# mahilab/mahi-mpc

Hardware: AMD Instinct MI355X
Metric: MPC solves/sec (whole node), nx=4 N=30 batch, at 1/2/4/8 MI355X (higher is better)
Workload: dtype f64; 1 GPU; cfg#2: 2-link arm nx=4 nu=2, N=30, h=2 ms, cold-start SQP (exact or Gauss-Newton Hessian: config.hessian) to ||grad||<=1e-8, ||g||<=1e-10; batch_per_gpu=4096, global_batch=4096, horizon=30, kkt_solver=riccati (16 lanes per instance), hessian=exact (Lagrangian, IPOPT's default), init_states=reference cold start V = 0 (MMPC_INIT_ZERO: V not read)

## Files before the change

### mahi-mpc_amd/csrc/sqp_group.h

```cpp
#undef MMPC_GROUP_PASS
#if defined(MMPC_GROUP_BODY_ONLY)
#define MMPC_GROUP_PASS 2
#elif !defined(MMPC_SQP_GROUP_H)
#define MMPC_SQP_GROUP_H
#define MMPC_GROUP_PASS 1
#else
#define MMPC_GROUP_PASS 0
#endif
#if MMPC_GROUP_PASS == 1
#include <type_traits>

#include "models.h"
#include "sqp_lane.h"
#include "sqp_wave.h"

namespace mmpc {

template <class Model>
__host__ __device__ constexpr bool w_struct_zero(int, int) { return false; }
template <>
__host__ __device__ constexpr bool w_struct_zero<TwoLinkArm>(int r, int j) { return (r == 0 && j >= 2) || (r >= 2 && (j == 0 || j >= 4)); }
template <class Model>
struct WPack {
    static constexpr int PK = 0, OVER = 0;
// ... 123 lines not shown
        for (int s = 0; s < (NQ > NA ? NQ : NA); ++s) {
            if (s < NA) t = fma(lFqd[i * NA + s], x[NQ + s] - lxs[NQ + s], t);
            if (s < NQ) t = fma(lFq[i * NQ + s], x[s] - lxs[s], t);
        }
#pragma unroll
        for (int c = 0; c < NU; ++c) t = fma(lFu[i * NU + c], u[c] - lus[c], t);
        xd[NQ + i] = t;
    }
    if (jac) {
#pragma unroll
        for (int i = 0; i < NA * NQ; ++i) Fq[i] = lFq[i];
#pragma unroll
        for (int i = 0; i < NA * NA; ++i) Fqd[i] = lFqd[i];
#pragma unroll
        for (int i = 0; i < NA * NU; ++i) Fu[i] = lFu[i];
    }
}

template <class Model, bool BOUNDED = false, bool XB = false, bool EXACT = false>
__global__ __launch_bounds__(64) void sqp_group_kernel(SolveParams p, GroupWork gw) {
    constexpr bool MEHR = false;
    constexpr bool IB = false;
#endif
#if MMPC_GROUP_PASS != 0
    static_assert(!(BOUNDED && XB), "the interior-point variant handles the control bounds itself");
    static_assert(!MEHR || XB, "the barrier rule belongs to the interior-point variant");
    constexpr int NX = Model::NX, NU = Model::NU, NQ = Model::NQ, NA = NX - NQ, NS = NX + NU, ND = NX + NU;
    constexpr int SQ = NA * NQ > 0 ? NA * NQ : 1;
    constexpr int FQ = NA * NQ, FD = NA * NA, FU = NA * NU;
    static_assert(NQ >= 0 && NA >= NQ, "x = [q; z] with qdot = z[0:NQ]");
    constexpr int G = kGroupLanes;
    extern __shared__ double shm[];
    const int gl = threadIdx.x & (G - 1);
    const int gi = threadIdx.x / G;
    [[maybe_unused]] const int lane0 = threadIdx.x;
    MMPC_PHASE_DECL
    const int gbase = gi * G;
    const int64_t slot = (int64_t)blockIdx.x * p.gpw + gi;
    const bool resume = p.tail_idx != nullptr;
    const bool valid = gi < p.gpw && slot < (resume ? (int64_t)min(*p.tail_count, p.tail_slots) : p.B);
    if (!valid) return;
    const int64_t inst = resume ? (int64_t)p.tail_idx[slot] : slot;
    const int64_t ii = inst;
    const int N = p.N;
    const int NV = NX * (N + 1) + NU * N;
    const double h = p.h;

    constexpr int KC = NX + NU < kGroupLanes ? GroupLaneOps<Model>::doubles : 0;
    double* const sX = shm + gi * group_lds_doubles(NX, NU, NQ, N, BOUNDED, p.is_linear != 0, XB, KC);
    double* const sU = sX + (N + 1) * NX;
    double* const sD = sU + N * NU;
    double* const sDX = sD + (N + 1) * NX;
    double* const sDU = sDX + (N + 1) * NX;
    double* const sF = sDU + N * NU;
    double* const sC = sF + N * NX;
    double* const sFq = sC + N * NX;
    double* const sFqd = sFq + N * FQ;
    double* const sFu = sFqd + N * FD;
    double* const sR = sFu + N * FU;
    double* const sHold = sR + N * NX;
    double* const sLin = sHold + (BOUNDED ? N * NU : 0);
    constexpr int NY = NX + NU;
    constexpr int PK = WPack<Model>::PK;
    constexpr bool WLDS = EXACT && !BOUNDED && !XB && IsControlAffine<Model>::value && PK >= NX && PK <= 2 * NX + NU;
    double* const wK = gw.ws + slot * (int64_t)group_ws_doubles(NX, NU, N, BOUNDED, XB, WLDS, MEHR);
    constexpr int KZ = NX + NU, HW = group_hess_doubles(NX, NU);
    double* const wH = wK + N * NU * (NS + 1);
    double* const sW = sD + NX;
    static_assert(!WLDS || WPack<Model>::OVER <= NX, "the over-read of the last W record stays inside sDU");
    if constexpr (WLDS) {
        if (gl < WPack<Model>::OVER) sW[N * PK + gl] = 0.0;
    }
    constexpr int NR = NS + NU + 1;
    double* const wRel = wH + N * HW;
    bool w_zeros_stored = false;
    double* const sZl = wRel;
    double* const sZu = sZl + N * NY;
    double* const sSg = sZu + N * NY;
    double* const sBb = sSg + N * NY;
    double* const sZg = sBb + N * NY;
    [[maybe_unused]] double* const sCl = sZg + N * NY;
    [[maybe_unused]] double* const sCu = sCl + N * NY;
    constexpr int VL = 2 + NU, VC = NU * (NU + 1) / 2, VS = VC + NU, VR = VL * G + VS;
    [[maybe_unused]] double* const sVr = sCu + N * NY;
    const double* const trg = p.traj + ii * (int64_t)N * NX;

    const double* w = p.weights + ii * p.w_stride;
    double Q[NX], R[NU], Rm[NU], up[NU];
#pragma unroll
    for (int r = 0; r < NX; ++r) Q[r] = w[r];
#pragma unroll
    for (int c = 0; c < NU; ++c) {
        R[c] = w[NX + c];
        Rm[c] = w[NX + NU + c];
        up[c] = p.u_prev[ii * NU + c];
    }
    double lbv[NU], ubv[NU];
    load_bounds<NU, BOUNDED, IB>(p, inst, lbv, ubv);
    constexpr bool DIST = (NS < G);
    static_assert(!MEHR || DIST, "Mehrotra's rule: lane-distributed path");
    constexpr bool CAFF = IsControlAffine<Model>::value;
    static_assert(!EXACT || (DIST && HasHess<Model>::value), "exact Hessian: lane-distributed path, model eval_hess");
    const int r = gl;
    const bool lx = r < NX, lu = r >= NX && r < NS, la = r >= NQ && r < NX;
    const int rx = lx ? r : 0;
    const int ru = lu ? r - NX : 0;
    const int ta = la ? r - NQ : 0;
    const double Qr = lx ? w[rx] : 0.0;
    [[maybe_unused]] const double lqd = r < NQ ? 1.0 : 0.0, lad = la ? 1.0 : 0.0;
    const double lxf = lx ? 1.0 : 0.0;
    int wrow = 0;
#pragma unroll
    for (int r2 = 0; r2 < NX; ++r2)
        if (lx && r == r2) wrow = WPack<Model>::col(r2);
    double wm[KZ];
#pragma unroll
    for (int j = 0; j < KZ; ++j) {
        bool nz = false;
#pragma unroll
        for (int r2 = 0; r2 < NX; ++r2)
            if (lx && r == r2 && WPack<Model>::idx(r2, j) >= 0) nz = true;
        wm[j] = wpack_col_rep<Model>(j) < j ? wm[wpack_col_rep<Model>(j)] : (nz ? 1.0 : 0.0);
    }
    const int rq = r < NQ ? r : 0;
    const double Rr = lu ? w[NX + ru] : 0.0;
    double dgx[NS];
#pragma unroll
    for (int j = 0; j < NS; ++j) dgx[j] = (lx && j == r) ? 1.0 : 0.0;
    double lbr = -INFINITY, ubr = INFINITY;
#pragma unroll
    for (int c = 0; c < NU; ++c)
        if (lu && ru == c) {
            lbr = lbv[c];
            ubr = ubv[c];
        }
    double hq[NQ > 0 ? NQ : 1], hrow[NX], qoh[NX], rdg[NU];
#pragma unroll
    for (int z = 0; z < NQ; ++z) hq[z] = (r == NQ + z) ? h : 0.0;
#pragma unroll
    for (int j = 0; j < NX; ++j) {
        hrow[j] = (r < NQ && j == NQ + r) ? h : 0.0;
        qoh[j] = (j == r) ? Qr : 0.0;
    }
#pragma unroll
    for (int c = 0; c < NU; ++c) rdg[c] = (r == NX + c) ? R[c] : 0.0;
    constexpr bool LOPS = KC > 0;
    double* const sKc = sX + group_lds_doubles(NX, NU, NQ, N, BOUNDED, p.is_linear != 0, XB, KC) - KC;
    using LdsB = const __attribute__((address_space(3))) char*;
    using LdsD = const __attribute__((address_space(3))) double*;
    const LdsB shb = (LdsB)shm;
    auto lds = [](LdsB b) { return *(LdsD)b; };
    auto pin = [](LdsB& b) { asm volatile("" : "+v"(b)); };
    [[maybe_unused]] const LdsB iKc = shb + 8 * (int)(sKc - shm), iKz = iKc + 8 * NX;
    [[maybe_unused]] const LdsB iAq = la ? shb + 8 * ((int)(sFq - shm) + ta * NQ) : (r < NQ ? iKc + 8 * ((NX - 1) - (NQ + r)) : iKz);
    [[maybe_unused]] const int zAq = la ? 8 * FQ : 0, zAd = la ? 8 * FD : 0, zBr = la ? 8 * FU : 0;
    [[maybe_unused]] const LdsB iAd = la ? shb + 8 * ((int)(sFqd - shm) + ta * NA) : (r < NQ ? iAq + 8 * NQ : iKz);
    [[maybe_unused]] const LdsB iBr = la ? shb + 8 * ((int)(sFu - shm) + ta * NU) : iKz;
    constexpr bool ACOLP = LOPS && NQ == NA && (NA - 1) * NA < KC;
    [[maybe_unused]] const int zAc = (la || r < NQ) ? 8 * FD : 0;
    [[maybe_unused]] const LdsB iAc = la ? shb + 8 * ((int)(sFqd - shm) + ta) : (r < NQ ? shb + 8 * ((int)(sFq - shm) + rq) : iKc),
                                iAcN = iAc + (N - 1) * zAc;
    if constexpr (LOPS) {
        for (int i = gl; i < KC; i += G) sKc[i] = (i == NX - 1) ? h : 0.0;
    }
    {
        const double* Vin = p.V + ii * (int64_t)NV;
        for (int k = gl; k <= N; k += G) {
#pragma unroll
            for (int r = 0; r < NX; ++r)
                sX[k * NX + r] = (k == 0 || p.init_hold) ? p.x0[ii * NX + r] : (p.init_zero ? 0.0 : Vin[k * ND + r]);
            if (k < N) {
#pragma unroll
                for (int c = 0; c < NU; ++c) {
                    const double v = p.init_zero ? 0.0 : Vin[k * ND + NX + c];
                    sU[k * NU + c] = BOUNDED ? proj(v, lbv[c], ubv[c]) : v;
                }
#pragma unroll
                for (int r = 0; r < NX; ++r) sR[k * NX + r] = trg[k * NX + r];
            }
        }
    }
    const double* const tr = sR;
    double yl[XB ? NY : 1], yu[XB ? NY : 1];
    double mub = (XB && resume) ? p.tail_mub[slot] : kIpMu0;
    if constexpr (XB) {
        load_ip_bounds<NX, NU, IB>(p, inst, yl, yu);
        __builtin_amdgcn_wave_barrier();
        if (resume) {
            const double* const lz = p.tail_lws + (inst >> 6) * p.tail_lws_block + (inst & 63);
            for (int k = gl; k < N; k += G) {
#pragma unroll
                for (int j = 0; j < NY; ++j) {
                    sZl[k * NY + j] = lz[((int64_t)k * p.tail_lws_ss + p.tail_lws_zl + j) * 64];
                    sZu[k * NY + j] = lz[((int64_t)k * p.tail_lws_ss + p.tail_lws_zl + NY + j) * 64];
                }
            }
        } else {
            for (int k = gl; k < N; k += G) {
#pragma unroll
                for (int j = 0; j < NY; ++j) {
                    double& y = j < NX ? sX[(k + 1) * NX + j] : sU[k * NU + j - NX];
                    y = ip_push(y, yl[j], yu[j]);
                    sZl[k * NY + j] = yl[j] > -INFINITY ? 1.0 : 0.0;
                    sZu[k * NY + j] = yu[j] < INFINITY ? 1.0 : 0.0;
                }
            }
        }
    }
    const bool lin = p.is_linear != 0;
    double* const lFq = sLin;
    double* const lFqd = lFq + FQ;
    double* const lFu = lFqd + FD;
    double* const lxd = lFu + FU;
    const double* const lxs = sX;
    if (lin && gl == 0) {
        double acc[NA], x[NX], Fq[SQ], Fqd[FD], Fu[FU];
#pragma unroll
        for (int r = 0; r < NX; ++r) x[r] = p.x0[ii * NX + r];
        Model::eval_acc_jac(x, up, acc, Fq, Fqd, Fu);
#pragma unroll
        for (int i = 0; i < FQ; ++i) lFq[i] = Fq[i];
#pragma unroll
        for (int i = 0; i < FD; ++i) lFqd[i] = Fqd[i];
#pragma unroll
        for (int i = 0; i < FU; ++i) lFu[i] = Fu[i];
#pragma unroll
        for (int i = 0; i < NQ; ++i) lxd[i] = x[NQ + i];
#pragma unroll
        for (int i = 0; i < NA; ++i) lxd[NQ + i] = acc[i];
    }
    __builtin_amdgcn_wave_barrier();
    int status = ST_MAX_ITER;
    int it = 0;
    double kkt = 0.0, mu = resume ? p.tail_mu[slot] : 0.0, pg_prev = (BOUNDED && resume) ? p.tail_mub[slot] : INFINITY;
    bool done = !valid;
    constexpr bool FUSE_FWD = true;
    bool fwd_ready = false;
    double J0n = 0.0, c1n = 0.0, cmaxn = 0.0;
    int nfn = 0;
    MMPC_PHASE(0);
    for (it = resume ? p.tail_it[slot] : 0; !done; ++it) {
        MMPC_PHASE(8);
        __builtin_amdgcn_wave_barrier();
        double J0 = J0n, c1 = c1n, cmax = cmaxn;
        int nonfinite = nfn;
        const bool evalA = !(FUSE_FWD && fwd_ready);
        if (evalA) {
            J0 = 0.0;
            c1 = 0.0;
            cmax = 0.0;
            nonfinite = 0;
            for (int k = gl; k < N; k += G) {
                double x[NX], u[NU], xd[NX], Fq[SQ], Fqd[FD], Fu[FU];
#pragma unroll
                for (int r = 0; r < NX; ++r) x[r] = sX[k * NX + r];
#pragma unroll
                for (int c = 0; c < NU; ++c) u[c] = sU[k * NU + c];
                group_model<Model>(lin, lFq, lFqd, lFu, lxd, lxs, up, x, u, xd, Fq, Fqd, Fu, true);
#pragma unroll
                for (int i = 0; i < FQ; ++i) sFq[k * FQ + i] = h * Fq[i];
#pragma unroll
                for (int i = 0; i < FD; ++i) sFqd[k * FD + i] = h * Fqd[i];
#pragma unroll
                for (int i = 0; i < FU; ++i) sFu[k * FU + i] = h * Fu[i];
#pragma unroll
                for (int r = 0; r < NX; ++r) {
                    const double F = fma(h, xd[r], x[r]);
                    sF[k * NX + r] = F;
                    const double c = F - sX[(k + 1) * NX + r];
                    sC[k * NX + r] = c;
                    cmax = fmax(cmax, fabs(c));
                    c1 += fabs(c);
                    nonfinite |= !isfinite(c);
                    const double e = F - tr[k * NX + r];
                    J0 = fma(e * Q[r], e, J0);
                }
#pragma unroll
                for (int c = 0; c < NU; ++c) {
                    const double um = (k == 0) ? up[c] : sU[(k - 1) * NU + c];
                    const double dif = u[c] - um;
                    J0 = fma(dif * R[c], dif, fma(u[c] * Rm[c], u[c], J0));
                }
            }
        }
        double lsum = 0.0, cmpl0 = 0.0, cmplmu = 0.0;
        if constexpr (XB) {
            for (int k = gl; k < N; k += G) {
#pragma unroll
                for (int j = 0; j < NY; ++j) {
                    const double y = j < NX ? sX[(k + 1) * NX + j] : sU[k * NU + j - NX];
                    double sg, bb, zg;
                    ip_terms(y, yl[j], yu[j], sZl[k * NY + j], sZu[k * NY + j], mub, sg, bb, zg, cmpl0, cmplmu, lsum);
                    sSg[k * NY + j] = sg;
                    if constexpr (MEHR) sBb[k * NY + j] = 0.0;
                    else sBb[k * NY + j] = bb;
                    sZg[k * NY + j] = zg;
                }
            }
            lsum = group_sum(lsum);
            cmpl0 = group_max(cmpl0);
            cmplmu = group_max(cmplmu);
            nonfinite |= !isfinite(lsum);
            __builtin_amdgcn_fence(__ATOMIC_RELEASE, "workgroup");
            __builtin_amdgcn_fence(__ATOMIC_ACQUIRE, "workgroup");
        }
        if (evalA) {
            J0 = group_sum(J0);
            c1 = group_sum(c1);
            cmax = group_max(cmax);
        }
        fwd_ready = false;
// ... 233 lines not shown
                            Y[a][j] = t * il[a];
                        }
#pragma unroll
                    for (int a = NU - 1; a >= 0; --a)
#pragma unroll
                        for (int j = 0; j <= NS; ++j) {
                            double t = Y[a][j];
#pragma unroll
                            for (int q = a + 1; q < NU; ++q) t = fma(-Ld[q][a], Kt[q][j], t);
                            Kt[a][j] = t * il[a];
                        }
                }
#pragma unroll
                for (int a = 0; a < NU; ++a)
#pragma unroll
                    for (int j = 0; j <= NS; ++j) wK[(k * NU + a) * (NS + 1) + j] = -Kt[a][j];
                if (k == 0) break;
                const double(&YB)[NU][NS + 1] = (NU == 2 && !XB) ? Kt : Y;
#pragma unroll
                for (int a = 0; a < NS; ++a) {
                    double t = pn[a];
#pragma unroll
                    for (int q = 0; q < NU; ++q) t = fma(-Y[q][a], YB[q][NS], t);
                    if (BOUNDED) t += pex[a];
                    pv[a] = t;
#pragma unroll
                    for (int b = a; b < NS; ++b) {
                        double v = (b < NX) ? Pn[a][b] : ((a == b) ? R[a - NX] : 0.0);
#pragma unroll
                        for (int q = 0; q < NU; ++q) v = fma(-Y[q][a], YB[q][b], v);
                        P[a][b] = v;
                    }
                }
            }
#undef Ps
        };
        double dJ = 0.0;
        bool resolve = false;
        auto step_sweep = [&](int pass) {
            dJ = 0.0;
            double dx[NX], dup[NU], um[NU];
#pragma unroll
            for (int r = 0; r < NX; ++r) {
                dx[r] = 0.0;
                sDX[r] = 0.0;
            }
#pragma unroll
            for (int c = 0; c < NU; ++c) {
                dup[c] = 0.0;
                um[c] = up[c];
            }
            constexpr int NK = NU * (NS + 1);
            double nK[NK], nFq[SQ], nFqd[FD], nFu[FU], nF[NX], nc[NX], nr[NX], nu_[NU];
#define GROUP_LOAD_STEP(k_)                                                                        \
        do {                                                                                           \
            const int kk_ = (k_);                                                                      \
            _Pragma("unroll") for (int i_ = 0; i_ < NK; ++i_) nK[i_] = wK[kk_ * NK + i_];              \
            _Pragma("unroll") for (int i_ = 0; i_ < FQ; ++i_) nFq[i_] = sFq[kk_ * FQ + i_];             \
            _Pragma("unroll") for (int i_ = 0; i_ < FD; ++i_) nFqd[i_] = sFqd[kk_ * FD + i_];           \
            _Pragma("unroll") for (int i_ = 0; i_ < FU; ++i_) nFu[i_] = sFu[kk_ * FU + i_];             \
            _Pragma("unroll") for (int r_ = 0; r_ < NX; ++r_) {                                        \
            nF[r_] = sF[kk_ * NX + r_];                                                            \
            nc[r_] = sC[kk_ * NX + r_];                                                            \
            nr[r_] = sR[kk_ * NX + r_];                                                            \
            }                                                                                          \
            _Pragma("unroll") for (int c_ = 0; c_ < NU; ++c_) nu_[c_] = sU[kk_ * NU + c_];             \
        } while (0)
            GROUP_LOAD_STEP(0);
            constexpr int kStepUnroll = NX <= 4 ? 2 : 1;
#pragma unroll kStepUnroll
            for (int k = 0; k < N; ++k) {
                double K[NK], hFq[SQ], hFqd[FD], hFu[FU], Fk[NX], ck[NX], rk[NX], uk[NU];
#pragma unroll
                for (int i = 0; i < NK; ++i) K[i] = nK[i];
#pragma unroll
                for (int i = 0; i < FQ; ++i) hFq[i] = nFq[i];
#pragma unroll
                for (int i = 0; i < FD; ++i) hFqd[i] = nFqd[i];
#pragma unroll
                for (int i = 0; i < FU; ++i) hFu[i] = nFu[i];
#pragma unroll
                for (int r = 0; r < NX; ++r) {
                    Fk[r] = nF[r];
                    ck[r] = nc[r];
                    rk[r] = nr[r];
                }
#pragma unroll
                for (int c = 0; c < NU; ++c) uk[c] = nu_[c];
                if (k + 1 < N) GROUP_LOAD_STEP(k + 1);
                double du[NU];
#pragma unroll
                for (int a = 0; a < NU; ++a) {
                    double t = K[a * (NS + 1) + NS];
#pragma unroll
                    for (int q = 0; q < NX; ++q) t = fma(K[a * (NS + 1) + q], dx[q], t);
#pragma unroll
                    for (int c = 0; c < NU; ++c) t = fma(K[a * (NS + 1) + NX + c], dup[c], t);
                    du[a] = t;
                    sDU[k * NU + a] = t;
                }
                if (BOUNDED && pass + 1 < kBoundPasses) {
#pragma unroll
                    for (int a = 0; a < NU; ++a) {
                        const double hv = sHold[k * NU + a], t = uk[a] + du[a];
                        if (hv != hv && (t < lbv[a] || t > ubv[a])) {
                            sHold[k * NU + a] = t < lbv[a] ? lbv[a] : ubv[a];
                            resolve = true;
                        }
                    }
                }
                double ad[NX];
                a_mul<NQ, NA, double>(h, hFq, hFqd, dx, ad);
#pragma unroll
                for (int s = 0; s < NA; ++s)
#pragma unroll
                    for (int c = 0; c < NU; ++c) ad[NQ + s] = fma(hFu[s * NU + c], du[c], ad[NQ + s]);
#pragma unroll
                for (int r = 0; r < NX; ++r) {
                    const double qe = 2.0 * Q[r] * (Fk[r] - rk[r]);
                    dJ = fma(qe, ad[r], dJ);
                    dx[r] = ad[r] + ck[r];
                    sDX[(k + 1) * NX + r] = dx[r];
                }
#pragma unroll
                for (int c = 0; c < NU; ++c) {
                    const double dif = uk[c] - um[c];
                    dJ = fma(2.0 * R[c] * dif, du[c] - dup[c], fma(2.0 * Rm[c] * uk[c], du[c], dJ));
                    um[c] = uk[c];
                    dup[c] = du[c];
                }
            }
#undef GROUP_LOAD_STEP
        };
        auto colA = [&](double own, const double* acol, const double* vb) {
            double t = lxf * own;
#pragma unroll
            for (int z = 0; z < NQ; ++z) t = fma(hq[z], vb[z], t);
#pragma unroll
            for (int s2 = 0; s2 < NA; ++s2) t = fma(acol[s2], vb[NQ + s2], t);
            return t;
        };
        auto load_arow = [&](int k, double* arow, double* brow) {
#pragma unroll
            for (int s2 = 0; s2 < NQ; ++s2)
                arow[s2] = LOPS ? lds(iAq + __mul24(k, zAq) + 8 * s2) : fma(lad, sFq[k * FQ + ta * NQ + s2], hrow[s2]);
#pragma unroll
            for (int s2 = 0; s2 < NA; ++s2)
                arow[NQ + s2] = LOPS ? lds(iAd + __mul24(k, zAd) + 8 * s2) : fma(lad, sFqd[k * FD + ta * NA + s2], hrow[NQ + s2]);
#pragma unroll
            for (int c = 0; c < NU; ++c) brow[c] = LOPS ? lds(iBr + __mul24(k, zBr) + 8 * c) : lad * sFu[k * FU + ta * NU + c];
        };
        auto d_recursion_dist = [&]() {
            double dr = 0.0;
            if (lx) sD[rx] = 0.0;
            struct Op {
                double q[NQ > 0 ? NQ : 1], d[NA], c;
            };
            LdsB jq = iAq, jd = iAd;
            auto fetch = [&](int k, Op& o) {
#pragma unroll
                for (int s2 = 0; s2 < NQ; ++s2) o.q[s2] = LOPS ? lds(jq + 8 * s2) : sFq[k * FQ + ta * NQ + s2];
#pragma unroll
                for (int s2 = 0; s2 < NA; ++s2) o.d[s2] = LOPS ? lds(jd + 8 * s2) : sFqd[k * FD + ta * NA + s2];
                o.c = sC[k * NX + rx];
                if constexpr (LOPS) {
                    jq += zAq;
                    jd += zAd;
                    pin(jq);
                    pin(jd);
                }
            };
            auto stage = [&](int k, Op& o) {
                double db[NX], arow[NX];
#pragma unroll
                for (int s2 = 0; s2 < NQ; ++s2) arow[s2] = LOPS ? o.q[s2] : fma(lad, o.q[s2], hrow[s2]);
#pragma unroll
                for (int s2 = 0; s2 < NA; ++s2) arow[NQ + s2] = LOPS ? o.d[s2] : fma(lad, o.d[s2], hrow[NQ + s2]);
                const double cr = o.c;
                fetch(k + 2, o);
                sfor<0, NX>([&](auto I) { db[I] = row_bcast<I>(dr); });
                double t0 = dr + cr, t1 = 0.0;
#pragma unroll
                for (int j = 0; j < NX; ++j) {
                    if (j & 1) t1 = fma(arow[j], db[j], t1);
                    else t0 = fma(arow[j], db[j], t0);
                }
                dr = t0 + t1;
                if (lx) sD[(k + 1) * NX + rx] = dr;
            };
            Op o0, o1;
            fetch(0, o0);
            fetch(LOPS || N > 1 ? 1 : 0, o1);
            int k = 0;
            for (; k + 1 < N; k += 2) {
                stage(k, o0);
                stage(k + 1, o1);
            }
            if (k < N) stage(k, o0);
        };
        auto load_acol = [&](int k, [[maybe_unused]] LdsB& jc, double* acol) {
            if constexpr (ACOLP) {
#pragma unroll
                for (int t2 = 0; t2 < NA; ++t2) acol[t2] = lds(jc + 8 * t2 * NA);
                jc -= zAc;
                pin(jc);
            } else {
#pragma unroll
                for (int t2 = 0; t2 < NA; ++t2) {
                    double v = lad * sFqd[k * FD + t2 * NA + ta];
                    if constexpr (NQ > 0) v = fma(lqd, sFq[k * FQ + t2 * NQ + rq], v);
                    acol[t2] = v;
                }
            }
        };
        auto adjoint_dist = [&]() {
            double lamr;
            {
                const double eb = lx ? sX[N * NX + rx] - tr[(N - 1) * NX + rx] : 0.0;
                lamr = Qr * (sD[N * NX + rx] + eb);
                if constexpr (XB) lamr += lxf * sZg[(N - 1) * NY + rx];
                lmax = fmax(lmax, fabs(lamr));
                if (lx) sD[N * NX + rx] = lamr;
            }
            struct Op {
                double fd[NA], fq[NA], xk, trm, dk, zg;
            };
            [[maybe_unused]] LdsB jc = iAcN;
            auto fetch = [&](int k, Op& o) {
#pragma unroll
                for (int t2 = 0; t2 < NA; ++t2) {
                    if constexpr (ACOLP) {
                        o.fd[t2] = lds(jc + 8 * t2 * NA);
                    } else {
                        o.fd[t2] = sFqd[k * FD + t2 * NA + ta];
                        if constexpr (NQ > 0) o.fq[t2] = sFq[k * FQ + t2 * NQ + rq];
                    }
                }
                if constexpr (ACOLP) {
                    jc -= zAc;
                    pin(jc);
                }
                o.xk = sX[k * NX + rx];
                o.trm = tr[(k - 1) * NX + rx];
                o.dk = sD[k * NX + rx];
                if constexpr (XB) o.zg = sZg[(k - 1) * NY + rx];
            };
            auto stage = [&](int k, Op& o) {
                double acol[NA];
#pragma unroll
                for (int t2 = 0; t2 < NA; ++t2) {
                    if constexpr (ACOLP) {
                        acol[t2] = o.fd[t2];
                    } else {
                        double v = lad * o.fd[t2];
                        if constexpr (NQ > 0) v = fma(lqd, o.fq[t2], v);
                        acol[t2] = v;
                    }
                }
                double qe = Qr * (o.dk + (o.xk - o.trm));
                if constexpr (XB) qe += o.zg;
                fetch(k >= 3 ? k - 2 : 1, o);
                double lamb[NX];
                sfor<0, NX>([&](auto I) { lamb[I] = row_bcast<I>(lamr); });
                double t0 = lamr + qe, t1 = 0.0;
#pragma unroll
                for (int z = 0; z < NQ; ++z) t1 = fma(hq[z], lamb[z], t1);
#pragma unroll
                for (int s2 = 0; s2 < NA; ++s2) {
                    if (s2 & 1) t1 = fma(acol[s2], lamb[NQ + s2], t1);
                    else t0 = fma(acol[s2], lamb[NQ + s2], t0);
                }
                lamr = t0 + t1;
                lmax = fmax(lmax, fabs(lxf * lamr));
                if (lx) sD[k * NX + rx] = lamr;
            };
            if (N >= 2) {
                Op o0, o1;
                fetch(N - 1, o0);
                fetch(N >= 3 ? N - 2 : 1, o1);
                int k = N - 1;
                for (; k >= 2; k -= 2) {
                    stage(k, o0);
                    stage(k - 1, o1);
                }
                if (k == 1) stage(1, o0);
            }
            __builtin_amdgcn_fence(__ATOMIC_RELEASE, "workgroup");
            __builtin_amdgcn_fence(__ATOMIC_ACQUIRE, "workgroup");
            for (int k = gl; k < N; k += G) {
#pragma unroll
                for (int c = 0; c < NU; ++c) {
                    double g = 0.0;
#pragma unroll
                    for (int s2 = 0; s2 < NA; ++s2) g = fma(sFu[k * FU + s2 * NU + c], sD[(k + 1) * NX + NQ + s2], g);
                    const double uk = sU[k * NU + c], um = k == 0 ? up[c] : sU[(k - 1) * NU + c];
                    g = fma(R[c], uk - um, fma(Rm[c], uk, g));
                    if (k < N - 1) g -= R[c] * (sU[(k + 1) * NU + c] - uk);
                    if constexpr (XB) g += sZg[k * NY + NX + c];
                    if constexpr (!BOUNDED) {
                        gmax = fmax(gmax, fabs(2.0 * g));
                    } else {
                        gmax = fmax(gmax, fabs(uk - proj(uk - 2.0 * g, lbv[c], ubv[c])));
                        sHold[k * NU + c] = (uk <= lbv[c] + beps && g > 0.0)   ? lbv[c]
                                            : (uk >= ubv[c] - beps && g < 0.0) ? ubv[c]
                                                                                : NAN;
                    }
                    nonfinite |= !isfinite(g);
                }
            }
        };
        auto backward_dist = [&](bool useW) {
            if constexpr (BOUNDED) {
                __builtin_amdgcn_fence(__ATOMIC_RELEASE, "workgroup");
                __builtin_amdgcn_fence(__ATOMIC_ACQUIRE, "workgroup");
            }
            double Prow[NS], pvr;
            [[maybe_unused]] LdsB jcol = iAcN;
            const double lxm = lx ? 1.0 : 0.0;
            struct Wb {
                double r[KZ], u[NU * NU];
            };
            Wb w0;
            auto load_w = [&](int k, Wb& b) {
#pragma unroll
                for (int j = 0; j < KZ; ++j)
                    b.r[j] = WLDS ? sW[k * PK + wrow + WPack<Model>::col(j)] : wH[k * HW + rx * KZ + j];
                if constexpr (!CAFF) {
#pragma unroll
                    for (int j = 0; j < NU * NU; ++j) b.u[j] = wH[k * HW + NX * KZ + j];
                }
            };
            if (EXACT && useW) {
                load_w(N - 1, w0);
            }
#pragma unroll
            for (int j = 0; j < NS; ++j) Prow[j] = j < NX ? qoh[j] : 0.0;
            pvr = Qr * (lx ? sX[N * NX + rx] - tr[(N - 1) * NX + rx] : 0.0);
            if constexpr (XB) {
                const double sgN = sSg[(N - 1) * NY + rx], bbN = sBb[(N - 1) * NY + rx];
#pragma unroll
                for (int j = 0; j < NX; ++j) Prow[j] = fma(dgx[j], sgN, Prow[j]);
                pvr = fma(lxm, bbN, pvr);
            }
            auto stage = [&](int k, auto last_c, Wb& wb) {
                constexpr bool LAST = decltype(last_c)::value;
#if defined(MMPC_PHASE_TIMING) && defined(MMPC_PHASE_STAGES)
                if (gl == 0 && blockIdx.x < kPhaseWavePhases && k < 32)
                    g_mmpc_phase_cycles[kPhaseStageLog + 128 * blockIdx.x + 32 * gi + k] = __builtin_amdgcn_s_memtime();
#endif
                double hFq[SQ], hFqd[FD], hFu[FU], cc[NX], u[NU], um[NU], acol[NA];
#pragma unroll
                for (int i = 0; i < FQ; ++i) hFq[i] = sFq[k * FQ + i];
#pragma unroll
                for (int i = 0; i < FD; ++i) hFqd[i] = sFqd[k * FD + i];
#pragma unroll
                for (int i = 0; i < FU; ++i) hFu[i] = sFu[k * FU + i];
#pragma unroll
                for (int q = 0; q < NX; ++q) cc[q] = sC[k * NX + q];
#pragma unroll
                for (int c = 0; c < NU; ++c) {
                    u[c] = sU[k * NU + c];
                    um[c] = LAST ? up[c] : sU[(k - 1) * NU + c];
                }
                load_acol(k, jcol, acol);
                double xsgu[XB ? NU : 1], xbbu[XB ? NU : 1], xsgx = 0.0, xbbx = 0.0;
                if constexpr (XB) {
#pragma unroll
                    for (int a = 0; a < NU; ++a) {
                        xsgu[a] = sSg[k * NY + NX + a];
                        xbbu[a] = sBb[k * NY + NX + a];
                    }
                    if constexpr (!LAST) {
                        xsgx = sSg[(k - 1) * NY + rx];
                        xbbx = sBb[(k - 1) * NY + rx];
                    }
                }
                double exr = 0.0, duu = 0.0;
                if constexpr (!LAST) {
                    const double xk = sX[k * NX + rx], trm = tr[(k - 1) * NX + rx];
                    exr = xk - trm;
                    duu = sU[k * NU + ru] - sU[(k - 1) * NU + ru];
                }
                double wr[KZ], wu[NU * NU];
                if constexpr (EXACT) {
#pragma unroll
                    for (int j = 0; j < KZ; ++j) wr[j] = useW ? wb.r[j] : 0.0;
#pragma unroll
                    for (int j = 0; j < NU * NU; ++j) wu[j] = (useW && !CAFF) ? wb.u[j] : 0.0;
                    if (!LAST && useW) load_w(k - 1, wb);
                }
                double T[NU], mv = pvr;
#pragma unroll
                for (int b = 0; b < NU; ++b) {
                    double t = Prow[NX + b];
#pragma unroll
                    for (int s2 = 0; s2 < NA; ++s2) t = fma(Prow[NQ + s2], hFu[s2 * NU + b], t);
                    T[b] = t;
                }
#pragma unroll
                for (int q = 0; q < NX; ++q) mv = fma(Prow[q], cc[q], mv);
                double Tb[NS][NU], mvb[NS];
                sfor<0, NS>([&](auto I) {
#pragma unroll
                    for (int b = 0; b < NU; ++b) Tb[I][b] = row_bcast<I>(T[b]);
                    mvb[I] = row_bcast<I>(mv);
                });
                double Hww[NU][NU], hw[NU];
#pragma unroll
                for (int a = 0; a < NU; ++a) {
#pragma unroll
                    for (int b = a; b < NU; ++b) {
                        double t = Tb[NX + a][b];
#pragma unroll
                        for (int s2 = 0; s2 < NA; ++s2) t = fma(hFu[s2 * NU + a], Tb[NQ + s2][b], t);
                        if (a == b) t += R[a] + Rm[a];
                        if constexpr (EXACT && !CAFF) t += wu[a * NU + b];
                        if constexpr (XB) {
                            if (a == b) t += xsgu[a];
                        }
                        Hww[a][b] = t;
                        Hww[b][a] = t;
                    }
                    double t = fma(R[a], u[a] - um[a], fma(Rm[a], u[a], mvb[NX + a]));
#pragma unroll
                    for (int s2 = 0; s2 < NA; ++s2) t = fma(hFu[s2 * NU + a], mvb[NQ + s2], t);
                    if constexpr (XB) t += xbbu[a];
                    hw[a] = t;
                }
                double Ycol[NU];
#pragma unroll
                for (int a = 0; a < NU; ++a) {
                    double tb[NX];
#pragma unroll
                    for (int q = 0; q < NX; ++q) tb[q] = Tb[q][a];
                    Ycol[a] = colA(T[a], acol, tb) - rdg[a];
                    if constexpr (EXACT) Ycol[a] = fma(WLDS ? wm[NX + a] : lxm, wr[NX + a], Ycol[a]);
                }
                if constexpr (BOUNDED) {
// ... 324 lines not shown
                    fetch(k >= 2 ? k - 2 : 0, o0);
                    stage(k - 1, o1);
                }
                if (k == 0) stage(0, o0);
            }
        };
        if constexpr (DIST) {
            d_recursion_dist();
            adjoint_dist();
            lmax = group_max(lmax);
            gmax = group_max(gmax);
        } else if (gl == 0) {
            {
                double d[NX];
#pragma unroll
                for (int r = 0; r < NX; ++r) {
                    d[r] = 0.0;
                    sD[r] = 0.0;
                }
                double aq[SQ], ad[FD], ac[NX];
#pragma unroll
                for (int i = 0; i < FQ; ++i) aq[i] = sFq[i];
#pragma unroll
                for (int i = 0; i < FD; ++i) ad[i] = sFqd[i];
#pragma unroll
                for (int r = 0; r < NX; ++r) ac[r] = sC[r];
                constexpr int kDUnroll = NX <= 4 ? 2 : 1;
#pragma unroll kDUnroll
                for (int k = 0; k < N; ++k) {
                    double fq[SQ], fd[FD], cc[NX], dn[NX];
#pragma unroll
                    for (int i = 0; i < FQ; ++i) fq[i] = aq[i];
#pragma unroll
                    for (int i = 0; i < FD; ++i) fd[i] = ad[i];
#pragma unroll
                    for (int r = 0; r < NX; ++r) cc[r] = ac[r];
                    const int kn = k + 1 < N ? k + 1 : k;
#pragma unroll
                    for (int i = 0; i < FQ; ++i) aq[i] = sFq[kn * FQ + i];
#pragma unroll
                    for (int i = 0; i < FD; ++i) ad[i] = sFqd[kn * FD + i];
#pragma unroll
                    for (int r = 0; r < NX; ++r) ac[r] = sC[kn * NX + r];
                    a_mul<NQ, NA, double>(h, fq, fd, d, dn);
#pragma unroll
                    for (int r = 0; r < NX; ++r) {
                        d[r] = dn[r] + cc[r];
                        sD[(k + 1) * NX + r] = d[r];
                    }
                }
            }
            backward(0);
        }
        if constexpr (!DIST) {
            gmax = group_bcast(gmax, gbase);
            lmax = group_bcast(lmax, gbase);
            fact_ok = group_bcast_i(fact_ok, gbase);
        }
        MMPC_PHASE(2);
        nonfinite = (group_max((double)nonfinite) != 0.0);
        kkt = fmax(gmax, cmax);
        if (XB) kkt = fmax(kkt, 2.0 * cmpl0);
        double* trc = p.trace && valid ? p.trace + (inst * (p.max_iter + 1) + it) * 8 : nullptr;
        if (trc && gl == 0) {
            trc[0] = gmax;
            trc[1] = cmax;
            trc[2] = J0;
            trc[3] = c1;
            trc[7] = lmax;
        }
        if (nonfinite || !isfinite(kkt)) {
            status = ST_NONFINITE;
            break;
        }
        if (gmax <= p.tol_grad && cmax <= p.tol_defect && (!XB || 2.0 * cmpl0 <= kIpTolCompl)) {
            status = ST_CONVERGED;
            break;
        }
        if (it == p.max_iter) {
            status = ST_MAX_ITER;
            break;
        }
        MMPC_PHASE(9);
        if constexpr (EXACT) {
            __builtin_amdgcn_wave_barrier();
            auto w_stage = [&](int k) {
                double x[NX], u[NU], la[NA], W[KZ * KZ];
#pragma unroll
                for (int r2 = 0; r2 < NX; ++r2) x[r2] = sX[k * NX + r2];
#pragma unroll
                for (int c = 0; c < NU; ++c) u[c] = sU[k * NU + c];
#pragma unroll
                for (int s2 = 0; s2 < NA; ++s2) la[s2] = h * sD[(k + 1) * NX + NQ + s2];
                if constexpr (WLDS) __builtin_amdgcn_wave_barrier();
                Model::eval_hess(x, u, la, W);
                if constexpr (WLDS) {
                    static_assert(!WLDS || PK >= NX, "write order of the W pass");
#pragma unroll
                    for (int r2 = 0; r2 < NX; ++r2)
#pragma unroll
                        for (int j = r2; j < KZ; ++j)
                            if (WPack<Model>::idx(r2, j) >= 0) sW[k * PK + WPack<Model>::idx(r2, j)] = W[r2 * KZ + j];
                } else {
                    double* const dst = wH + k * HW;
#pragma unroll
                    for (int r2 = 0; r2 < NX; ++r2)
#pragma unroll
                        for (int j = 0; j < KZ; ++j)
                            if (!w_struct_zero<Model>(r2, j) || !w_zeros_stored) dst[r2 * KZ + j] = W[r2 * KZ + j];
                    if constexpr (!CAFF) {
#pragma unroll
                        for (int a = 0; a < NU; ++a)
#pragma unroll
                            for (int b = 0; b < NU; ++b) dst[NX * KZ + a * NU + b] = W[(NX + a) * KZ + NX + b];
                    }
                }
            };
            if constexpr (WLDS) {
                for (int k0 = ((N - 1) / G) * G; k0 >= 0; k0 -= G)
                    if (k0 + gl < N) w_stage(k0 + gl);
                MMPC_PHASE(9);
                __builtin_amdgcn_wave_barrier();
            } else {
                for (int k = gl; k < N; k += G) w_stage(k);
                w_zeros_stored = true;
                MMPC_PHASE(9);
                __builtin_amdgcn_fence(__ATOMIC_RELEASE, "workgroup");
                __builtin_amdgcn_fence(__ATOMIC_ACQUIRE, "workgroup");
            }
        }
        bool use_w = EXACT;
        if constexpr (DIST) {
            backward_dist(use_w);
            if (EXACT && !fact_ok) {
                fact_ok = 1;
                use_w = false;
                backward_dist(false);
            }
        }
        if (!fact_ok) {
            status = ST_FACT_FAILED;
            break;
        }
        if (BOUNDED) pg_prev = gmax;
        const double mub_next = (XB && fmax(fmax(0.5 * gmax, cmax), cmplmu) <= kIpKappaEps * mub)
                                    ? fmax(kIpTolCompl / 20.0, fmin(kIpKappaMu * mub, pow(mub, kIpThetaMu)))
                                    : mub;

        MMPC_PHASE(3);
        if constexpr (DIST) {
            auto step_dist = [&](bool check) {
                __builtin_amdgcn_fence(__ATOMIC_RELEASE, "workgroup");
                __builtin_amdgcn_fence(__ATOMIC_ACQUIRE, "workgroup");
                double sr = 0.0;
                if (lx) sDX[rx] = 0.0;
                constexpr int NK = NS + 1;
                const double* const Kp = wK + ru * NK;
                struct Ops {
                    double K[NK], a[NX], b[NU], c, Rw[BOUNDED ? NR : 1];
                };
                const double* const Rp = wRel + ru * NR;
                auto fetch = [&](int k, Ops& o) {
#pragma unroll
                    for (int j = 0; j < NK; ++j) o.K[j] = Kp[k * NU * NK + j];
                    load_arow(k, o.a, o.b);
                    o.c = sC[k * NX + rx];
                    if constexpr (BOUNDED) {
#pragma unroll
                        for (int j = 0; j < NR; ++j) o.Rw[j] = Rp[k * NU * NR + j];
                    }
                };
                auto stage = [&](int k, Ops& o) {
                    double sb[NS];
                    sfor<0, NS>([&](auto I) { sb[I] = row_bcast<I>(sr); });
                    double du0 = o.K[NS], du1 = 0.0;
#pragma unroll
                    for (int j = 0; j < NS; ++j) {
                        if (j & 1) du1 = fma(o.K[j], sb[j], du1);
                        else du0 = fma(o.K[j], sb[j], du0);
                    }
                    const double du = du0 + du1;
                    double ad = sr;
#pragma unroll
                    for (int j = 0; j < NX; ++j) ad = fma(o.a[j], sb[j], ad);
                    double dub[NU];
                    sfor<0, NU>([&](auto I) { dub[I] = row_bcast<NX + I>(du); });
#pragma unroll
                    for (int c = 0; c < NU; ++c) ad = fma(o.b[c], dub[c], ad);
                    const double dxn = ad + o.c;
                    if (lx) {
                        sDX[(k + 1) * NX + rx] = dxn;
                        sD[(k + 1) * NX + rx] = ad;
                    }
                    if (lu) sDU[k * NU + ru] = du;
                    if constexpr (BOUNDED) {
                        if (check && lu) {
                            const double hv = sHold[k * NU + ru], t = sU[k * NU + ru] + du;
                            if (hv != hv) {
                                if (t < lbr || t > ubr) {
                                    sHold[k * NU + ru] = t < lbr ? lbr : ubr;
                                    resolve = true;
                                }
                            } else if (!p.no_release) {
                                double m = o.Rw[NR - 1];
#pragma unroll
                                for (int j = 0; j < NS; ++j) m = fma(o.Rw[j], sb[j], m);
#pragma unroll
                                for (int b = 0; b < NU; ++b) m = fma(o.Rw[NS + b], dub[b], m);
                                if ((hv == lbr && m < 0.0) || (hv == ubr && m > 0.0)) {
                                    sHold[k * NU + ru] = NAN;
                                    resolve = true;
                                }
                            }
                        }
                    }
                    sr = lx ? dxn : (lu ? du : 0.0);
                    fetch(k + 3 < N ? k + 3 : N - 1, o);
                };
                Ops o0, o1, o2;
                fetch(0, o0);
                fetch(N > 1 ? 1 : 0, o1);
                fetch(N > 2 ? 2 : 0, o2);
                if (N % 3 == 1) {
                    stage(0, o0);
                    for (int k = 1; k < N; k += 3) {
                        stage(k, o1);
                        stage(k + 1, o2);
                        stage(k + 2, o0);
                    }
                } else if (N % 3 == 2) {
                    stage(0, o0);
                    stage(1, o1);
                    for (int k = 2; k < N; k += 3) {
                        stage(k, o2);
                        stage(k + 1, o0);
                        stage(k + 2, o1);
                    }
                } else {
                    for (int k = 0; k < N; k += 3) {
                        stage(k, o0);
                        stage(k + 1, o1);
                        stage(k + 2, o2);
                    }
                }
            };
            if constexpr (MEHR) {
                step_dist(false);
                __builtin_amdgcn_wave_barrier();
                double ap = 1.0, ad = 1.0, sz = 0.0;
                for (int k = gl; k < N; k += G) {
#pragma unroll
                    for (int j = 0; j < NY; ++j) {
                        const double y = j < NX ? sX[(k + 1) * NX + j] : sU[k * NU + j - NX];
                        const double dy = j < NX ? sDX[(k + 1) * NX + j] : sDU[k * NU + j - NX];
                        ip_aff_limits(y, dy, yl[j], yu[j], sZl[k * NY + j], sZu[k * NY + j], ap, ad, sz);
                    }
                }
                ap = group_min(ap);
                ad = group_min(ad);
                sz = group_sum(sz);
                double saff = 0.0;
                for (int k = gl; k < N; k += G) {
#pragma unroll
                    for (int j = 0; j < NY; ++j) {
                        const double y = j < NX ? sX[(k + 1) * NX + j] : sU[k * NU + j - NX];
                        const double dy = j < NX ? sDX[(k + 1) * NX + j] : sDU[k * NU + j - NX];
                        saff += ip_aff_compl(y, dy, yl[j], yu[j], sZl[k * NY + j], sZu[k * NY + j], ap, ad);
                    }
                }
                saff = group_sum(saff);
                int nb = 0;
#pragma unroll
                for (int j = 0; j < NY; ++j) nb += (yl[j] > -INFINITY) + (yu[j] < INFINITY);
                const double mbnd = (double)nb * (double)N;
                const double muc = sz / mbnd, mua = saff / mbnd;
                const double sig = muc > 0.0 ? pow(mua / muc, 3.0) : 0.0;
                mub = fmax(kIpTolCompl / 20.0, fmin(sig * muc, kIpMu0));
                for (int k = gl; k < N; k += G) {
#pragma unroll
                    for (int j = 0; j < NY; ++j) {
                        const double y = j < NX ? sX[(k + 1) * NX + j] : sU[k * NU + j - NX];
                        const double dy = j < NX ? sDX[(k + 1) * NX + j] : sDU[k * NU + j - NX];
                        double ccl, ccu, bb;
                        ip_corrector(y, dy, yl[j], yu[j], sZl[k * NY + j], sZu[k * NY + j], mub, ccl, ccu, bb);
                        sCl[k * NY + j] = ccl;
                        sCu[k * NY + j] = ccu;
                        sBb[k * NY + j] = bb;
                    }
                }
                __builtin_amdgcn_fence(__ATOMIC_RELEASE, "workgroup");
                __builtin_amdgcn_fence(__ATOMIC_ACQUIRE, "workgroup");
                backward_vec();
            }
            for (int pass = 0;; ++pass) {
                if (pass > 0) {
                    __builtin_amdgcn_fence(__ATOMIC_RELEASE, "workgroup");
                    __builtin_amdgcn_fence(__ATOMIC_ACQUIRE, "workgroup");
                    backward_dist(use_w);
                    if (EXACT && use_w && !fact_ok) {
                        fact_ok = 1;
                        use_w = false;
                        backward_dist(false);
                    }
                    if (!fact_ok) break;
                }
                resolve = false;
                const int passes = (it == 0 && !p.no_release) ? 2 : kBoundPasses;
                step_dist(BOUNDED && pass + 1 < passes);
                if constexpr (!BOUNDED) {
                    break;
                } else {
                    resolve = group_max(resolve ? 1.0 : 0.0) != 0.0;
                    if (!resolve || pass + 1 >= passes) break;
                }
            }
            __builtin_amdgcn_wave_barrier();
            double dj = 0.0;
            for (int k = gl; k < N; k += G) {
#pragma unroll
                for (int q = 0; q < NX; ++q) dj = fma(2.0 * Q[q] * (sF[k * NX + q] - tr[k * NX + q]), sD[(k + 1) * NX + q], dj);
#pragma unroll
                for (int c = 0; c < NU; ++c) {
                    const double uk = sU[k * NU + c], duk = sDU[k * NU + c];
                    const double um = (k == 0) ? up[c] : sU[(k - 1) * NU + c];
                    const double dum = (k == 0) ? 0.0 : sDU[(k - 1) * NU + c];
                    dj = fma(2.0 * R[c] * (uk - um), duk - dum, fma(2.0 * Rm[c] * uk, duk, dj));
                }
            }
            dJ = group_sum(dj);
        } else {
            if (gl == 0) {
                for (int pass = 0;; ++pass) {
                    if (pass > 0) backward(pass);
                    if (!fact_ok) break;
                    resolve = false;
                    step_sweep(pass);
                    if (!BOUNDED || !resolve || pass + 1 >= kBoundPasses) break;
                }
            }
            fact_ok = group_bcast_i(fact_ok, gbase);
            dJ = group_bcast(dJ, gbase);
        }
        if (!fact_ok) {
            status = ST_FACT_FAILED;
            break;
        }
        __builtin_amdgcn_wave_barrier();
        MMPC_PHASE(4);
        double amax = 1.0, az = 1.0, dbar = 0.0;
        if constexpr (XB) {
            const double tau = kIpTau;
            for (int k = gl; k < N; k += G) {
#pragma unroll
                for (int j = 0; j < NY; ++j) {
                    const double y = j < NX ? sX[(k + 1) * NX + j] : sU[k * NU + j - NX];
                    const double dy = j < NX ? sDX[(k + 1) * NX + j] : sDU[k * NU + j - NX];
                    if constexpr (MEHR)
                        ip_step_limits_pc(y, dy, yl[j], yu[j], sZl[k * NY + j], sZu[k * NY + j], mub, tau,
                                          sCl[k * NY + j], sCu[k * NY + j], amax, az, dbar);
                    else
                        ip_step_limits(y, dy, yl[j], yu[j], sZl[k * NY + j], sZu[k * NY + j], mub, tau, sBb[k * NY + j],
                                       amax, az, dbar);
                }
            }
            amax = group_min(amax);
            az = group_min(az);
            dbar = group_sum(dbar);
        }

        mu = fmax(mu, 4.0 * lmax + 1.0);
        const double phi0 = XB ? fma(mu, c1, fma(-2.0 * mub, lsum, J0)) : fma(mu, c1, J0);
        const double dphi = XB ? dJ + dbar - mu * c1 : dJ - mu * c1;
// ... 177 lines not shown
```

Measured before the change: 27.45 million solves/s.

## Mirror idle lanes onto state rows and stream operands via pointer-walk prefetch

Adds a MIRROR mode for models with NQ==NA and a cached Kc column. In this mode, lanes that do not own a state row run the same recursion as a mirrored state row, so their stores and loads become unconditional and the per-lane predication goes away. The forward distance, adjoint and step recursions now place operand prefetches after a scheduling barrier. The step recursion walks incrementing LDS and global pointers instead of recomputing indexed addresses. The aim is to cut address arithmetic and branch divergence on the serial horizon recursions. The cost is redundant lane work, duplicate writes to shared memory, and more register pressure from the extra pointers.

```diff
diff --git a/mahi-mpc_amd/csrc/sqp_group.h b/mahi-mpc_amd/csrc/sqp_group.h
--- a/mahi-mpc_amd/csrc/sqp_group.h
+++ b/mahi-mpc_amd/csrc/sqp_group.h
@@ -299,11 +299,15 @@
     auto lds = [](LdsB b) { return *(LdsD)b; };
     auto pin = [](LdsB& b) { asm volatile("" : "+v"(b)); };
     [[maybe_unused]] const LdsB iKc = shb + 8 * (int)(sKc - shm), iKz = iKc + 8 * NX;
-    [[maybe_unused]] const LdsB iAq = la ? shb + 8 * ((int)(sFq - shm) + ta * NQ) : (r < NQ ? iKc + 8 * ((NX - 1) - (NQ + r)) : iKz);
+    constexpr bool MIRROR = LOPS && NQ > 0 && NQ == NA && (NA - 1) * NA < KC;
+    [[maybe_unused]] const double Qa = MIRROR ? w[rx] : Qr;
+    [[maybe_unused]] const LdsB iAq =
+        la ? shb + 8 * ((int)(sFq - shm) + ta * NQ) : ((r < NQ || MIRROR) ? iKc + 8 * ((NX - 1) - (NQ + rq)) : iKz);
     [[maybe_unused]] const int zAq = la ? 8 * FQ : 0, zAd = la ? 8 * FD : 0, zBr = la ? 8 * FU : 0;
-    [[maybe_unused]] const LdsB iAd = la ? shb + 8 * ((int)(sFqd - shm) + ta * NA) : (r < NQ ? iAq + 8 * NQ : iKz);
+    [[maybe_unused]] const LdsB iAd = la ? shb + 8 * ((int)(sFqd - shm) + ta * NA) : ((r < NQ || MIRROR) ? iAq + 8 * NQ : iKz);
     [[maybe_unused]] const LdsB iBr = la ? shb + 8 * ((int)(sFu - shm) + ta * NU) : iKz;
     constexpr bool ACOLP = LOPS && NQ == NA && (NA - 1) * NA < KC;
+    static_assert(!MIRROR || ACOLP, "a mirrored lane reads row 0's column through the per-lane column address");
     [[maybe_unused]] const int zAc = (la || r < NQ) ? 8 * FD : 0;
     [[maybe_unused]] const LdsB iAc = la ? shb + 8 * ((int)(sFqd - shm) + ta) : (r < NQ ? shb + 8 * ((int)(sFq - shm) + rq) : iKc),
                                 iAcN = iAc + (N - 1) * zAc;
@@ -843,7 +847,7 @@
         };
         auto d_recursion_dist = [&]() {
             double dr = 0.0;
-            if (lx) sD[rx] = 0.0;
+            if (MIRROR || lx) sD[rx] = 0.0;
             struct Op {
                 double q[NQ > 0 ? NQ : 1], d[NA], c;
             };
@@ -868,7 +872,7 @@
 #pragma unroll
                 for (int s2 = 0; s2 < NA; ++s2) arow[NQ + s2] = LOPS ? o.d[s2] : fma(lad, o.d[s2], hrow[NQ + s2]);
                 const double cr = o.c;
-                fetch(k + 2, o);
+                if constexpr (!MIRROR) fetch(k + 2, o);
                 sfor<0, NX>([&](auto I) { db[I] = row_bcast<I>(dr); });
                 double t0 = dr + cr, t1 = 0.0;
 #pragma unroll
@@ -877,7 +881,11 @@
                     else t0 = fma(arow[j], db[j], t0);
                 }
                 dr = t0 + t1;
-                if (lx) sD[(k + 1) * NX + rx] = dr;
+                if (MIRROR || lx) sD[(k + 1) * NX + rx] = dr;
+                if constexpr (MIRROR) {
+                    __builtin_amdgcn_sched_barrier(0);
+                    fetch(k + 2, o);
+                }
             };
             Op o0, o1;
             fetch(0, o0);
@@ -907,16 +915,17 @@
         auto adjoint_dist = [&]() {
             double lamr;
             {
-                const double eb = lx ? sX[N * NX + rx] - tr[(N - 1) * NX + rx] : 0.0;
-                lamr = Qr * (sD[N * NX + rx] + eb);
-                if constexpr (XB) lamr += lxf * sZg[(N - 1) * NY + rx];
+                const double eb = (MIRROR || lx) ? sX[N * NX + rx] - tr[(N - 1) * NX + rx] : 0.0;
+                lamr = Qa * (sD[N * NX + rx] + eb);
+                if constexpr (XB) lamr += (MIRROR ? 1.0 : lxf) * sZg[(N - 1) * NY + rx];
                 lmax = fmax(lmax, fabs(lamr));
-                if (lx) sD[N * NX + rx] = lamr;
+                if (MIRROR || lx) sD[N * NX + rx] = lamr;
             }
             struct Op {
                 double fd[NA], fq[NA], xk, trm, dk, zg;
             };
-            [[maybe_unused]] LdsB jc = iAcN;
+            [[maybe_unused]] LdsB jc = (!MIRROR || lx) ? iAcN : shb + 8 * ((int)(sFq - shm) + (N - 1) * FD);
+            [[maybe_unused]] const int zc = MIRROR ? 8 * FD : zAc;
             auto fetch = [&](int k, Op& o) {
 #pragma unroll
                 for (int t2 = 0; t2 < NA; ++t2) {
@@ -928,7 +937,7 @@
                     }
                 }
                 if constexpr (ACOLP) {
-                    jc -= zAc;
+                    jc -= zc;
                     pin(jc);
                 }
                 o.xk = sX[k * NX + rx];
@@ -936,7 +945,7 @@
                 o.dk = sD[k * NX + rx];
                 if constexpr (XB) o.zg = sZg[(k - 1) * NY + rx];
             };
-            auto stage = [&](int k, Op& o) {
+            auto stage = [&](int k, Op& o, [[maybe_unused]] bool more = true) {
                 double acol[NA];
 #pragma unroll
                 for (int t2 = 0; t2 < NA; ++t2) {
@@ -948,9 +957,9 @@
                         acol[t2] = v;
                     }
                 }
-                double qe = Qr * (o.dk + (o.xk - o.trm));
+                double qe = Qa * (o.dk + (o.xk - o.trm));
                 if constexpr (XB) qe += o.zg;
-                fetch(k >= 3 ? k - 2 : 1, o);
+                if constexpr (!MIRROR) fetch(k >= 3 ? k - 2 : 1, o);
                 double lamb[NX];
                 sfor<0, NX>([&](auto I) { lamb[I] = row_bcast<I>(lamr); });
                 double t0 = lamr + qe, t1 = 0.0;
@@ -962,19 +971,40 @@
                     else t0 = fma(acol[s2], lamb[NQ + s2], t0);
                 }
                 lamr = t0 + t1;
-                lmax = fmax(lmax, fabs(lxf * lamr));
-                if (lx) sD[k * NX + rx] = lamr;
+                lmax = fmax(lmax, fabs(MIRROR ? lamr : lxf * lamr));
+                if (MIRROR || lx) sD[k * NX + rx] = lamr;
+                if constexpr (MIRROR) {
+                    __builtin_amdgcn_sched_barrier(0);
+                    if (more) fetch(k - 2, o);
+                }
             };
             if (N >= 2) {
                 Op o0, o1;
                 fetch(N - 1, o0);
                 fetch(N >= 3 ? N - 2 : 1, o1);
                 int k = N - 1;
-                for (; k >= 2; k -= 2) {
-                    stage(k, o0);
-                    stage(k - 1, o1);
-                }
-                if (k == 1) stage(1, o0);
+                if constexpr (MIRROR) {
+                    for (; k >= 4; k -= 2) {
+                        stage(k, o0);
+                        stage(k - 1, o1);
+                    }
+                    if (k == 3) {
+                        stage(3, o0);
+                        stage(2, o1, false);
+                        stage(1, o0, false);
+                    } else if (k == 2) {
+                        stage(2, o0, false);
+                        stage(1, o1, false);
+                    } else {
+                        stage(1, o0, false);
+                    }
+                } else {
+                    for (; k >= 2; k -= 2) {
+                        stage(k, o0);
+                        stage(k - 1, o1);
+                    }
+                    if (k == 1) stage(1, o0);
+                }
             }
             __builtin_amdgcn_fence(__ATOMIC_RELEASE, "workgroup");
             __builtin_amdgcn_fence(__ATOMIC_ACQUIRE, "workgroup");
@@ -1605,14 +1635,54 @@
             auto step_dist = [&](bool check) {
                 __builtin_amdgcn_fence(__ATOMIC_RELEASE, "workgroup");
                 __builtin_amdgcn_fence(__ATOMIC_ACQUIRE, "workgroup");
+                constexpr bool RUN = MIRROR;
                 double sr = 0.0;
-                if (lx) sDX[rx] = 0.0;
+                if (RUN || lx) sDX[rx] = 0.0;
                 constexpr int NK = NS + 1;
                 const double* const Kp = wK + ru * NK;
                 struct Ops {
                     double K[NK], a[NX], b[NU], c, Rw[BOUNDED ? NR : 1];
                 };
                 const double* const Rp = wRel + ru * NR;
+                using LdsW = __attribute__((address_space(3))) double*;
+                [[maybe_unused]] LdsB ja = iAq, jd = iAd, jb = iBr, jcs = shb + 8 * ((int)(sC - shm) + rx);
+                [[maybe_unused]] LdsB js = shb + 8 * (lu ? (int)(sDU - shm) + ru : (int)(sDX - shm) + NX + rx);
+                [[maybe_unused]] LdsB jt = shb + 8 * (lu ? (int)(sD - shm) + ru : (int)(sD - shm) + NX + rx);
+                [[maybe_unused]] const int zs = lu ? 8 * NU : 8 * NX, zt = lu ? 0 : 8 * NX;
+                using GlbD = const __attribute__((address_space(1))) double*;
+                [[maybe_unused]] GlbD jK = (GlbD)Kp;
+                [[maybe_unused]] GlbD jR = (GlbD)Rp;
+                [[maybe_unused]] auto refill = [&](Ops& o) {
+#pragma unroll
+                    for (int j = 0; j < NK; ++j) o.K[j] = jK[j];
+#pragma unroll
+                    for (int s2 = 0; s2 < NQ; ++s2) o.a[s2] = lds(ja + 8 * s2);
+#pragma unroll
+                    for (int s2 = 0; s2 < NA; ++s2) o.a[NQ + s2] = lds(jd + 8 * s2);
+#pragma unroll
+                    for (int c = 0; c < NU; ++c) o.b[c] = lds(jb + 8 * c);
+                    o.c = lds(jcs);
+                    if constexpr (BOUNDED) {
+#pragma unroll
+                        for (int j = 0; j < NR; ++j) o.Rw[j] = jR[j];
+                    }
+                };
+                [[maybe_unused]] auto advance = [&]() {
+                    ja += zAq;
+                    jd += zAd;
+                    jb += zBr;
+                    jcs += 8 * NX;
+                    jK += NU * NK;
+                    pin(ja);
+                    pin(jd);
+                    pin(jb);
+                    pin(jcs);
+                    asm volatile("" : "+v"(jK));
+                    if constexpr (BOUNDED) {
+                        jR += NU * NR;
+                        asm volatile("" : "+v"(jR));
+                    }
+                };
                 auto fetch = [&](int k, Ops& o) {
 #pragma unroll
                     for (int j = 0; j < NK; ++j) o.K[j] = Kp[k * NU * NK + j];
@@ -1623,7 +1693,7 @@
                         for (int j = 0; j < NR; ++j) o.Rw[j] = Rp[k * NU * NR + j];
                     }
                 };
-                auto stage = [&](int k, Ops& o) {
+                auto stage = [&](int k, Ops& o, [[maybe_unused]] bool more = true) {
                     double sb[NS];
                     sfor<0, NS>([&](auto I) { sb[I] = row_bcast<I>(sr); });
                     double du0 = o.K[NS], du1 = 0.0;
@@ -1641,11 +1711,21 @@
 #pragma unroll
                     for (int c = 0; c < NU; ++c) ad = fma(o.b[c], dub[c], ad);
                     const double dxn = ad + o.c;
-                    if (lx) {
-                        sDX[(k + 1) * NX + rx] = dxn;
-                        sD[(k + 1) * NX + rx] = ad;
-                    }
-                    if (lu) sDU[k * NU + ru] = du;
+                    if constexpr (RUN) {
+                        sr = lu ? du : dxn;
+                        *(LdsW)js = sr;
+                        *(LdsW)jt = ad;
+                        js += zs;
+                        jt += zt;
+                        pin(js);
+                        pin(jt);
+                    } else {
+                        if (lx) {
+                            sDX[(k + 1) * NX + rx] = dxn;
+                            sD[(k + 1) * NX + rx] = ad;
+                        }
+                        if (lu) sDU[k * NU + ru] = du;
+                    }
                     if constexpr (BOUNDED) {
                         if (check && lu) {
                             const double hv = sHold[k * NU + ru], t = sU[k * NU + ru] + du;
@@ -1667,10 +1747,49 @@
                             }
                         }
                     }
-                    sr = lx ? dxn : (lu ? du : 0.0);
-                    fetch(k + 3 < N ? k + 3 : N - 1, o);
+                    if constexpr (RUN) {
+                        if (more) {
+                            refill(o);
+                            advance();
+                        }
+                    } else {
+                        sr = lx ? dxn : (lu ? du : 0.0);
+                        fetch(k + 3 < N ? k + 3 : N - 1, o);
+                    }
                 };
                 Ops o0, o1, o2;
+                if constexpr (RUN) {
+                    refill(o0);
+                    if (N > 1) advance();
+                    refill(o1);
+                    if (N > 2) advance();
+                    refill(o2);
+                    advance();
+                    int k = 0;
+                    for (; k + 5 < N; k += 3) {
+                        stage(k, o0, true);
+                        stage(k + 1, o1, true);
+                        stage(k + 2, o2, true);
+                    }
+                    const int left = N - 3 - k;
+                    if (left == 1) {
+                        stage(k, o0, true);
+                        stage(k + 1, o1, false);
+                        stage(k + 2, o2, false);
+                        stage(k + 3, o0, false);
+                    } else if (left == 2) {
+                        stage(k, o0, true);
+                        stage(k + 1, o1, true);
+                        stage(k + 2, o2, false);
+                        stage(k + 3, o0, false);
+                        stage(k + 4, o1, false);
+                    } else {
+                        stage(k, o0, false);
+                        if (N >= 2) stage(k + 1, o1, false);
+                        if (N >= 3) stage(k + 2, o2, false);
+                    }
+                    return;
+                }
                 fetch(0, o0);
                 fetch(N > 1 ? 1 : 0, o1);
                 fetch(N > 2 ? 2 : 0, o2);
```

After: 29.84 million solves/s, median of 6. 1.09x the previous value.
